# integritychain/fips204

Measured on AMD Instinct MI355X. Metric: ML-DSA-65 verifies/sec per GPU (batched); % HBM roofline, higher is better.
Workload: dtype int32; 1 GPU; ml_dsa_65 batch=65536 whole verify on FIPS 204 wire formats; batch_per_gpu=65536, parallelism=batch-split x1

## Files before the change

### fips204_amd/vfy/vfy.hip

```cpp
#include <hip/hip_runtime.h>
#include <stdint.h>
#include <string.h>

#include <mutex>
#include <string>
#include <vector>

#include "../../include/mldsa_vfy.h"
#include "../layer/layer_dev.h"
#include "../layer/layer_host.h"
#include "../csrc/challenge_dev.h"
#include "../csrc/ntt_wave.h"
#include "../csrc/sampler_dev.h"
#include "../csrc/tables.h"
#include "../csrc/verify_dev.h"
#include "keccak180.h"
#include "vfy_parts.h"

namespace mldsa_vfy {

using mldsa::FWD_TW;
using mldsa::INV_TW;
using mldsa::N;
using mldsa::SHAKE256_RATE;
using mldsa::SWAVES;
using mldsa::Twiddle;
using mldsa::load_le32;
using mldsa::static_for;

#ifndef MLDSA_VFY_EA_WAVES
#define MLDSA_VFY_EA_WAVES 5
#endif
template <int K, int L>
__global__ __launch_bounds__(64 * SWAVES) __attribute__((amdgpu_waves_per_eu(MLDSA_VFY_EA_WAVES, MLDSA_VFY_EA_WAVES))) void k_expand_a(const uint8_t* __restrict__ rho, size_t rho_stride,
                                                                                                    const uint32_t* __restrict__ key_idx,
                                                                                                    int32_t* __restrict__ a_hat, size_t n_ops,
                                                                                                    uint32_t n_keys) {
    const int lane = threadIdx.x & 63;
    const size_t g = (size_t)blockIdx.x * (64 * SWAVES) + threadIdx.x;
    const size_t wave_base = g - lane;
    const size_t n_streams = n_ops * (size_t)(K * L);
    const bool valid = g < n_streams;
    const size_t op = valid ? g / (K * L) : 0;
    const int rs = valid ? (int)(g % (K * L)) : 0;
    const int r = rs / L, sidx = rs % L;
    KeccakState st;
    size_t key = key_idx ? key_idx[op] : op;
    if (n_keys && key >= n_keys) key = 0;
    mldsa::expand_a_seed(st, rho + key * rho_stride, sidx, r);
    rej_ntt_poly_lane_direct180(st, a_hat, wave_base, lane, valid);
}

__global__ __launch_bounds__(256) void k_unpack_a(const uint32_t* __restrict__ packed, int32_t* __restrict__ out, size_t n_polys) {
    const size_t poly = (size_t)blockIdx.x * 4 + (threadIdx.x >> 6);
    if (poly >= n_polys) return;
    const int lane = threadIdx.x & 63;
    const uint32_t* p = packed + poly * mldsa::PACKED_POLY_DWORDS + 3 * lane;
    reinterpret_cast<int4*>(out + poly * N)[lane] = mldsa::unpack24(mldsa::Packed3{p[0], p[1], p[2]});
}

__global__ __launch_bounds__(256) void k_sanitize_keys(const uint32_t* __restrict__ key_idx, uint32_t n_keys, size_t n_ops,
                                                       uint32_t* __restrict__ safe, int32_t* __restrict__ bad) {
    const size_t i = (size_t)blockIdx.x * 256 + threadIdx.x;
    if (i >= n_ops) return;
    const uint32_t k = key_idx[i];
    safe[i] = k < n_keys ? k : 0u;
    bad[i] = k < n_keys ? 0 : 2;
}

constexpr int MU_BLK_STRIDE = 35;
__global__ __launch_bounds__(64) void k_mu(const uint8_t* __restrict__ tr, size_t tr_stride, const uint32_t* __restrict__ key_idx, int mode,
                                           const uint8_t* __restrict__ msgs, const uint64_t* __restrict__ msg_off,
                                           const uint8_t* __restrict__ ctxs, const uint64_t* __restrict__ ctx_off, uint8_t* __restrict__ mu,
                                           size_t mu_stride, int32_t* __restrict__ ctx_bad, const int32_t* __restrict__ key_bad, size_t n_ops,
                                           size_t op0, size_t n_call) {
    __shared__ uint32_t blk[64 * MU_BLK_STRIDE];
    const int lane = threadIdx.x;
    const size_t op = (size_t)blockIdx.x * 64 + lane;
    const bool valid = op < n_ops;
    uint32_t* row = blk + lane * MU_BLK_STRIDE;
    uint8_t* rowb = reinterpret_cast<uint8_t*>(row);

    const uint8_t *trp = nullptr, *mp = nullptr, *cp = nullptr;
    size_t mlen = 0, clen = 0;
    bool live = false;
    if (valid) {
        trp = tr + (key_idx ? key_idx[op] : op) * tr_stride;
        const uint64_t m0 = msg_off[op0 + op], m1 = msg_off[op0 + op + 1];
        bool bad_off = !(msg_off[0] <= m0 && m0 <= m1 && m1 <= msg_off[n_call]);
        mp = msgs + m0;
        mlen = (size_t)(m1 - m0);
        bad_off |= mlen != 0 && msgs == nullptr;
        if (ctx_off) {
            const uint64_t c0 = ctx_off[op0 + op], c1 = ctx_off[op0 + op + 1];
            bad_off |= !(ctx_off[0] <= c0 && c0 <= c1 && c1 <= ctx_off[n_call]);
            cp = ctxs + c0;
            clen = (size_t)(c1 - c0);
            bad_off |= clen != 0 && ctxs == nullptr;
        }
        const int flag = bad_off ? 2 : clen > 255 ? 1 : (key_bad ? key_bad[op] : 0);
        ctx_bad[op] = flag;
        live = !bad_off && clen <= 255;
        if (!live) mlen = clen = 0;
    }
    const size_t pre = (mode == MLDSA_MODE_INTERNAL) ? 0 : 2 + clen;
    const size_t total = live ? 64 + pre + mlen : 0;
    const size_t my_blocks = live ? total / SHAKE256_RATE + 1 : 0;
    size_t max_blocks = my_blocks;
#pragma unroll
    for (int m = 32; m >= 1; m >>= 1) {
        const size_t o = (size_t)__shfl_xor((unsigned long long)max_blocks, m);
        max_blocks = o > max_blocks ? o : max_blocks;
    }
    KeccakState st;
    mldsa::keccak_zero(st);
    for (size_t b = 0; b < max_blocks; b++) {
        if (b < my_blocks) {
            const size_t base = b * SHAKE256_RATE;
            auto byte_at = [&](size_t pos) -> uint8_t {
                if (pos < total) {
                    if (pos < 64) return trp[pos];
                    if (pos < 64 + pre) {
                        const size_t q = pos - 64;
                        return q == 0 ? (uint8_t)(mode == MLDSA_MODE_PREHASH ? 1 : 0) : q == 1 ? (uint8_t)clen : cp[q - 2];
                    }
                    return mp[pos - 64 - pre];
                }
                return pos == total ? (uint8_t)0x1F : (uint8_t)0;
            };
            for (int i = 0; i < SHAKE256_RATE / 4; i++) {
                const size_t pos = base + 4 * (size_t)i;
                uint32_t v;
                if (pos + 4 <= 64) v = load_le32(trp + pos);
                else if (pos >= 64 + pre && pos + 4 <= total) v = load_le32(mp + (pos - 64 - pre));
                else if (pos > total) v = 0;
                else v = (uint32_t)byte_at(pos) | ((uint32_t)byte_at(pos + 1) << 8) | ((uint32_t)byte_at(pos + 2) << 16) | ((uint32_t)byte_at(pos + 3) << 24);
                row[i] = v;
            }
            if (b == my_blocks - 1) rowb[SHAKE256_RATE - 1] |= 0x80;
            static_for<0, 17>([&](auto wc) {
                constexpr int W = decltype(wc)::value;
                st.lo[W] ^= row[2 * W];
                st.hi[W] ^= row[2 * W + 1];
            });
            mldsa::keccak_f1600(st);
        }
    }
    if (valid) {
        uint32_t* out = reinterpret_cast<uint32_t*>(mu + op * mu_stride);
#pragma unroll
        for (int i = 0; i < 8; i++) {
            out[2 * i] = st.lo[i];
            out[2 * i + 1] = st.hi[i];
        }
    }
}

template <int CT>
__global__ __launch_bounds__(64) void k_sample_in_ball(const uint8_t* __restrict__ c_tilde, size_t ct_stride, int tau, uint32_t* __restrict__ c_out,
                                                       size_t n_ops) {
    __shared__ uint32_t c_lds[64 * mldsa::SIB_C_STRIDE];
    __shared__ uint32_t b_lds[64 * mldsa::SIB_BLK_STRIDE];
    const int lane = threadIdx.x;
    const size_t wave_base = (size_t)blockIdx.x * 64;
    const size_t op = wave_base + lane;
    const bool valid = op < n_ops;
    KeccakState st;
    mldsa::keccak_zero(st);
    if (valid) mldsa::absorb_words<CT / 8>(st, c_tilde + op * ct_stride);
    mldsa::shake_pad<SHAKE256_RATE, CT>(st);
    mldsa::sample_in_ball_lane(st, tau, valid, c_lds + lane * mldsa::SIB_C_STRIDE, b_lds + lane * mldsa::SIB_BLK_STRIDE);
    mldsa::wave_lds_sync();
    for (int row = 0; row < 64; row++) {
        if (wave_base + row >= n_ops) break;
        const uint8_t* cb = reinterpret_cast<const uint8_t*>(c_lds + row * mldsa::SIB_C_STRIDE);
        c_out[(wave_base + row) * 64 + lane] =
            (uint32_t)cb[lane] | ((uint32_t)cb[64 + lane] << 8) | ((uint32_t)cb[128 + lane] << 16) | ((uint32_t)cb[192 + lane] << 24);
    }
}

template <int CTRL>
__device__ __forceinline__ int32_t dpp_all(int32_t v) {
    return __builtin_amdgcn_update_dpp(0, v, CTRL, 0xF, 0xF, true);
}

template <int M>
__device__ __forceinline__ void swap_pair(int32_t& x, int32_t& y, int lane) {
    if constexpr (M >= 4) {
        mldsa::swap_pair<M>(x, y, lane);
    } else {
        constexpr int CTRL = M == 2 ? 0x4E : 0xB1;
        const int32_t px = dpp_all<CTRL>(x), py = dpp_all<CTRL>(y);
        const bool up = (lane & M) != 0;
        x = up ? py : x;
        y = up ? y : px;
    }
}
template <int M>
__device__ __forceinline__ void xchg_hi(int32_t r[4], int lane) {
    swap_pair<M>(r[0], r[2], lane);
    swap_pair<M>(r[1], r[3], lane);
}
template <int M>
__device__ __forceinline__ void xchg_lo(int32_t r[4], int lane) {
    swap_pair<M>(r[0], r[1], lane);
    swap_pair<M>(r[2], r[3], lane);
}

template <class TW>
__device__ __forceinline__ void ntt_fwd_wave(int32_t r[4], const TW& tw, int lane) {
    using mldsa::bf_ct;
    bf_ct(r[0], r[2], mldsa::ZF1);
    bf_ct(r[1], r[3], mldsa::ZF1);
    bf_ct(r[0], r[1], mldsa::ZF2);
    bf_ct(r[2], r[3], mldsa::ZF3);
    xchg_hi<32>(r, lane);
    bf_ct(r[0], r[2], tw.get(0));
    bf_ct(r[1], r[3], tw.get(1));
    xchg_lo<16>(r, lane);
    bf_ct(r[0], r[1], tw.get(2));
    bf_ct(r[2], r[3], tw.get(3));
    xchg_hi<8>(r, lane);
    bf_ct(r[0], r[2], tw.get(4));
    bf_ct(r[1], r[3], tw.get(5));
    xchg_lo<4>(r, lane);
    bf_ct(r[0], r[1], tw.get(6));
    bf_ct(r[2], r[3], tw.get(7));
    xchg_hi<2>(r, lane);
    bf_ct(r[0], r[2], tw.get(8));
    bf_ct(r[1], r[3], tw.get(9));
    xchg_lo<1>(r, lane);
    bf_ct(r[0], r[1], tw.get(10));
    bf_ct(r[2], r[3], tw.get(11));
}
template <class TW>
__device__ __forceinline__ void ntt_inv_wave(int32_t r[4], const TW& tw, int lane, int32_t f) {
    using mldsa::bf_gs;
    bf_gs(r[0], r[1], tw.get(0));
    bf_gs(r[2], r[3], tw.get(1));
    bf_gs(r[0], r[2], tw.get(2));
    bf_gs(r[1], r[3], tw.get(3));
    xchg_lo<1>(r, lane);
    bf_gs(r[0], r[1], tw.get(4));
    bf_gs(r[2], r[3], tw.get(5));
    xchg_hi<2>(r, lane);
    bf_gs(r[0], r[2], tw.get(6));
    bf_gs(r[1], r[3], tw.get(7));
    xchg_lo<4>(r, lane);
    bf_gs(r[0], r[1], tw.get(8));
    bf_gs(r[2], r[3], tw.get(9));
    xchg_hi<8>(r, lane);
    bf_gs(r[0], r[2], tw.get(10));
    bf_gs(r[1], r[3], tw.get(11));
    xchg_lo<16>(r, lane);
    bf_gs(r[0], r[1], tw.get(12));
    bf_gs(r[2], r[3], tw.get(13));
    xchg_hi<32>(r, lane);
    const int32_t zf = (int32_t)((((int64_t)mldsa::ZI1 * f) % mldsa::Q) * mldsa::RINV_MOD_Q % mldsa::Q);
#pragma unroll
    for (int k = 0; k < 2; k++) {
        const int32_t a = r[k], b = r[k + 2];
        r[k] = mldsa::caddq(mldsa::mont_mul(a + b, f));
        r[k + 2] = mldsa::caddq(mldsa::mont_mul(a - b, zf));
    }
}

template <bool G2HI>
__device__ __forceinline__ void pack_w1_strided(const uint32_t v[4], uint8_t* dst, int lane) {
    if constexpr (G2HI) {
        uint32_t d[4];
#pragma unroll
        for (int k = 0; k < 4; k++) d[k] = v[k] << (4 * (lane & 7));
#pragma unroll
        for (int k = 0; k < 4; k++) d[k] |= (uint32_t)dpp_all<0xB1>((int32_t)d[k]);
#pragma unroll
        for (int k = 0; k < 4; k++) d[k] |= (uint32_t)dpp_all<0x4E>((int32_t)d[k]);
        const uint32_t d01 = (lane & 1) ? d[1] : d[0], d23 = (lane & 1) ? d[3] : d[2];
        uint32_t mine = (lane & 2) ? d23 : d01;
        mine |= (uint32_t)__builtin_amdgcn_update_dpp(0, (int32_t)mine, 0x104, 0xF, 0xF, true);
        if (!(lane & 4)) mldsa::store_row(reinterpret_cast<uint32_t*>(dst) + 8 * (lane & 3) + (lane >> 3), mine);
    } else {
#pragma unroll
        for (int k = 0; k < 4; k++) {
            const uint32_t n1 = (uint32_t)dpp_all<0xB1>((int32_t)v[k]);
            const uint32_t pair = (lane & 1) ? 0u : (v[k] | (n1 << 6));
            const uint32_t n2 = (uint32_t)dpp_all<0x4E>((int32_t)pair);
            if (!(lane & 3)) {
                const uint32_t q24 = pair | (n2 << 12);
                uint8_t* d = dst + 48 * k + 3 * (lane >> 2);
                d[0] = (uint8_t)q24; d[1] = (uint8_t)(q24 >> 8); d[2] = (uint8_t)(q24 >> 16);
            }
        }
    }
}

constexpr int VW = 4;
template <int K, int L, int GB, bool G2HI, int MINW>
__global__ __launch_bounds__(64 * VW) __attribute__((amdgpu_waves_per_eu(MINW))) void k_verify_main(
    const uint32_t* __restrict__ a_hat, const uint8_t* __restrict__ sigs, size_t sig_len, int ctilde_len, const uint32_t* __restrict__ c,
    const int32_t* __restrict__ t1, const uint32_t* __restrict__ key_idx, size_t key_base, int32_t* __restrict__ hvalid, int omega,
    uint8_t* __restrict__ w1, size_t w1_stride, int32_t* __restrict__ znorm, int32_t zbound, size_t n_ops, const Twiddle* __restrict__ fwd_tab,
    const Twiddle* __restrict__ inv_tab) {
    using mldsa::Packed3;
    constexpr int CB = GB + 1;
    constexpr int BITS = G2HI ? 4 : 6;
    __shared__ int4 zh[VW][L + 1][64];
    __shared__ uint32_t hint_lds[VW][mldsa::HINT_LDS_DWORDS];
    __shared__ Twiddle tw_lds[(FWD_TW + INV_TW) * 64];
    const int lane = threadIdx.x & 63;
    const int wave = __builtin_amdgcn_readfirstlane(threadIdx.x >> 6);
    for (int i = threadIdx.x; i < FWD_TW * 64; i += 64 * VW) tw_lds[i] = fwd_tab[i];
    for (int i = threadIdx.x; i < INV_TW * 64; i += 64 * VW) tw_lds[FWD_TW * 64 + i] = inv_tab[i];
    __syncthreads();
    const mldsa::LdsTw ftw{tw_lds, lane};
    const mldsa::LdsTw itw{tw_lds + FWD_TW * 64, lane};
    const uint32_t wid = blockIdx.x * VW + wave, n_waves = gridDim.x * VW;

    for (size_t op = wid; op < n_ops; op += n_waves) {
        unsigned ul = (unsigned)lane;
        asm volatile("" : "+v"(ul));
        const size_t key = key_idx ? (size_t)__builtin_amdgcn_readfirstlane((int)key_idx[op]) : key_base + op;
        const Packed3* arow = reinterpret_cast<const Packed3*>(a_hat + (op * K * (size_t)L) * mldsa::PACKED_POLY_DWORDS);
        const int4* trow = reinterpret_cast<const int4*>(t1 + (key * K) * (size_t)N);
        Packed3 av[L];
#pragma unroll
        for (int j = 0; j < L; j++) av[j] = mldsa::load_row<mldsa::NT_A_VERIFY>(&arow[(unsigned)(j * 64) + ul]);
        int4 tv = trow[ul];
        const uint8_t* zsrc = sigs + op * sig_len + ctilde_len;
        const mldsa::HintBytes hbytes = mldsa::hint_load(zsrc + L * (32 * CB), omega, K, (int)ul);
        bool zbad = false;
#pragma unroll 1
        for (int j = 0; j <= L; j++) {
            asm volatile("" ::: "memory");
            int32_t r[4];
            if (j < L) {
                const uint8_t* src = zsrc + (size_t)j * (32 * CB);
                int32_t mx = 0;
#pragma unroll
                for (int k = 0; k < 4; k++) {
                    r[k] = mldsa::y_from_raw<CB>(mldsa::y_raw_dword<CB, mldsa::NT_ZC>(src, k, (int)ul), (int)ul);
                    const int32_t a = r[k] < 0 ? -r[k] : r[k];
                    mx = a > mx ? a : mx;
                }
                zbad |= mx >= zbound;
            } else {
                const uint32_t d = mldsa::load_once<mldsa::NT_ZC>(c + op * 64 + ul);
                r[0] = (int8_t)(d & 0xFF); r[1] = (int8_t)((d >> 8) & 0xFF); r[2] = (int8_t)((d >> 16) & 0xFF); r[3] = (int8_t)(d >> 24);
            }
            mldsa_vfy::ntt_fwd_wave(r, ftw, lane);
            if (j == L) {
#pragma unroll
                for (int k = 0; k < 4; k++) r[k] = mldsa::mont_mul(r[k], -1);
            }
            zh[wave][j][lane] = make_int4(r[0], r[1], r[2], r[3]);
        }
        const bool hint_ok = mldsa::hint_unpack_wave<K>(hbytes, omega, hint_lds[wave], (int)ul);
        if (lane == 0) {
            znorm[op] = __ballot(zbad) != 0ull ? 0x7fffffff : 0;
            hvalid[op] = hint_ok ? 1 : 0;
        }
        auto row = [&](int i, const Packed3 (&a_cur)[L], const int4& t_cur, Packed3 (&a_nxt)[L], int4& t_nxt, bool more) {
            const int4 cv = zh[wave][L][lane];
            int64_t acc64[4] = {(int64_t)cv.x * t_cur.x, (int64_t)cv.y * t_cur.y, (int64_t)cv.z * t_cur.z, (int64_t)cv.w * t_cur.w};
#pragma unroll
            for (int j = 0; j < L; j++) {
                const int4 zv = zh[wave][j][lane];
                const int4 a4 = mldsa::unpack24(a_cur[j]);
                acc64[0] += (int64_t)a4.x * zv.x;
                acc64[1] += (int64_t)a4.y * zv.y;
                acc64[2] += (int64_t)a4.z * zv.z;
                acc64[3] += (int64_t)a4.w * zv.w;
            }
            int32_t acc[4];
            if (more) {
#pragma unroll
                for (int j = 0; j < L; j++) a_nxt[j] = mldsa::load_row<mldsa::NT_A_VERIFY>(&arow[(unsigned)(((i + 1) * L + j) * 64) + ul]);
                t_nxt = trow[(unsigned)((i + 1) * 64) + ul];
            }
#pragma unroll
            for (int k = 0; k < 4; k++) acc[k] = mldsa::mont_reduce64(acc64[k]);
            mldsa_vfy::ntt_inv_wave(acc, itw, lane, mldsa::F_MONT2);
            const uint32_t* hrow = hint_lds[wave] + 24 + i * 8 + (ul >> 5);
            uint8_t* dst = w1 + op * w1_stride + (size_t)i * (32 * BITS);
            uint32_t v[4];
#pragma unroll
            for (int k = 0; k < 4; k++) {
                const uint32_t h = (hrow[2 * k] >> (ul & 31)) & 1u;
                v[k] = (uint32_t)mldsa::use_hint<G2HI>((int32_t)h, acc[k]);
            }
            pack_w1_strided<G2HI>(v, dst, lane);
        };
        static_assert(K % 2 == 0, "the row loop runs two rows a trip");
        Packed3 aw[L];
        int4 tw2;
#pragma unroll 1
        for (int i = 0; i < K; i += 2) {
            asm volatile("" ::: "memory");
            row(i, av, tv, aw, tw2, true);
            asm volatile("" ::: "memory");
            row(i + 1, aw, tw2, av, tv, i + 2 < K);
        }
    }
}

constexpr int CWAVES = 4;
constexpr int CBLOCK = 64 * CWAVES;
template <int OUT>
__global__ __launch_bounds__(CBLOCK) void k_ctilde_verdict(const uint8_t* __restrict__ mu_w1, size_t mw, const uint8_t* __restrict__ sigs, size_t sig_len,
                                                           const int32_t* __restrict__ znorm, int32_t zbound, const int32_t* __restrict__ hvalid,
                                                           const int32_t* __restrict__ ctx_bad, uint8_t* __restrict__ ok, size_t n_ops) {
    __shared__ uint32_t tiles[CWAVES * 64 * mldsa::H_STRIDE];
    __shared__ unsigned long long ptr_a[CWAVES * 64];
    const int lane = threadIdx.x & 63, wave = threadIdx.x >> 6;
    uint32_t* tile = tiles + wave * 64 * mldsa::H_STRIDE;
    const size_t base_op = (size_t)blockIdx.x * CBLOCK;
    if (base_op >= n_ops) return;
    const size_t op = base_op + threadIdx.x;
    const bool valid = op < n_ops;
    const size_t opc = valid ? op : base_op;
    ptr_a[wave * 64 + lane] = (unsigned long long)(mu_w1 + opc * mw);
    mldsa::wave_lds_sync_c();
    KeccakState st;
    mldsa::shake256_2_absorb<true>(st, tile, ptr_a + wave * 64, ptr_a + wave * 64, (int)mw, 0, 0, 0, lane);
    if (!valid) return;
    const uint8_t* c0 = sigs + op * sig_len;
    uint32_t diff = 0;
    static_for<0, OUT / 8>([&](auto wc) {
        constexpr int W = decltype(wc)::value;
        diff |= (st.lo[W] ^ load_le32(c0 + 8 * W)) | (st.hi[W] ^ load_le32(c0 + 8 * W + 4));
    });
    ok[op] = (uint8_t)(diff == 0 && znorm[op] < zbound && hvalid[op] && !ctx_bad[op]);
}

}

namespace {

using namespace mldsa_layer;
using namespace mldsa_vfy;

struct DevState {
    int dev = -1;
    int n_cu = 256;
    hipStream_t ea = nullptr, vm = nullptr;
    std::vector<hipEvent_t> ev;
    Twiddle *fwd = nullptr, *inv = nullptr;
    bool prof_on = false;
    std::vector<hipEvent_t> prof_ev;
    std::vector<const char*> prof_name;
    size_t prof_used = 0;
};

std::mutex g_mutex;
std::vector<DevState*> g_states;
size_t g_part_ops = 0;

size_t part_ops() { return g_part_ops ? g_part_ops : (size_t)MLDSA_VFY_PART_OPS; }

int dev_state(const char* fn, int dev, DevState** out) {
    for (DevState* d : g_states)
        if (d->dev == dev) {
            *out = d;
            return MLDSA_OK;
        }
    DevState* d = new DevState;
    d->dev = dev;
    int cu = 0;
    if (hipDeviceGetAttribute(&cu, hipDeviceAttributeMultiprocessorCount, dev) == hipSuccess && cu > 0) d->n_cu = cu;
    const std::vector<mldsa::HostTwiddle> f = mldsa::gen_fwd_lane_twiddles(), i = mldsa::gen_inv_lane_twiddles();
    hipError_t e = hipStreamCreateWithFlags(&d->ea, hipStreamNonBlocking);
    if (e == hipSuccess) e = hipStreamCreateWithFlags(&d->vm, hipStreamNonBlocking);
    if (e == hipSuccess) e = hipMalloc(&d->fwd, f.size() * sizeof(Twiddle));
    if (e == hipSuccess) e = hipMalloc(&d->inv, i.size() * sizeof(Twiddle));
    if (e == hipSuccess) e = hipMemcpy(d->fwd, f.data(), f.size() * sizeof(Twiddle), hipMemcpyHostToDevice);
    if (e == hipSuccess) e = hipMemcpy(d->inv, i.data(), i.size() * sizeof(Twiddle), hipMemcpyHostToDevice);
    if (e != hipSuccess || f.size() != (size_t)FWD_TW * 64 || i.size() != (size_t)INV_TW * 64) {
        if (d->ea) (void)hipStreamDestroy(d->ea);
        if (d->vm) (void)hipStreamDestroy(d->vm);
        if (d->fwd) (void)hipFree(d->fwd);
        if (d->inv) (void)hipFree(d->inv);
        delete d;
        (void)hipGetLastError();
        return e != hipSuccess ? hip_failed(fn, "creating the library's streams and tables", e)
                               : fail(MLDSA_ERR_DEVICE, std::string(fn) + ": the core's twiddle tables have another shape");
    }
    g_states.push_back(d);
    *out = d;
    return MLDSA_OK;
}

struct Events {
    DevState* d;
    size_t used = 0;
    hipError_t err = hipSuccess;
    explicit Events(DevState* d_) : d(d_) {}
    hipEvent_t next() {
        if (used == d->ev.size()) {
            hipEvent_t e = nullptr;
            const hipError_t rc = hipEventCreateWithFlags(&e, hipEventDisableTiming);
            if (rc != hipSuccess) {
                err = rc;
                return nullptr;
            }
            d->ev.push_back(e);
        }
        return d->ev[used++];
    }
};

constexpr size_t PROF_MAX_PAIRS = 4096;
struct ProfScope {
    DevState* d;
    hipStream_t s;
    long idx = -1;
    ProfScope(DevState* d_, hipStream_t s_, const char* name) : d(d_), s(s_) {
        if (!d->prof_on || d->prof_used >= PROF_MAX_PAIRS) return;
        if (d->prof_used * 2 + 2 > d->prof_ev.size()) {
            hipEvent_t a = nullptr, b = nullptr;
            if (hipEventCreate(&a) != hipSuccess) return;
            if (hipEventCreate(&b) != hipSuccess) {
                (void)hipEventDestroy(a);
                return;
            }
            d->prof_ev.push_back(a);
            d->prof_ev.push_back(b);
            d->prof_name.push_back(name);
        } else {
            d->prof_name[d->prof_used] = name;
        }
        idx = (long)d->prof_used++;
        (void)hipEventRecord(d->prof_ev[2 * idx], s);
    }
    ~ProfScope() {
        if (idx >= 0) (void)hipEventRecord(d->prof_ev[2 * idx + 1], s);
    }
};

#define VFY_HIP(call, what)                                     \
    do {                                                        \
        const hipError_t e_ = (call);                           \
        if (e_ != hipSuccess) return hip_failed(fn, what, e_);  \
    } while (0)

#define VFY_BY_SET(set, M)              \
    do {                                \
        if ((set) == MLDSA_44) M(4, 4, 17, false, 32, 5); \
        else if ((set) == MLDSA_65) M(6, 5, 19, true, 48, 4); \
        else M(8, 7, 19, true, 64, 4);  \
    } while (0)

unsigned stream_blocks(size_t n_streams) { return (unsigned)((n_streams + 64 * SWAVES - 1) / (64 * SWAVES)); }

void launch_expand_a(int set, const uint8_t* rho, const uint32_t* key_idx, int32_t* a_hat, size_t n, uint32_t n_keys, hipStream_t s) {
    mldsa_params p;
    (void)mldsa_get_params(set, &p);
    const dim3 grid(stream_blocks(n * (size_t)(p.k * p.l))), block(64 * SWAVES);
#define VFY_EA(KK, LL, GB, G2, CT, MW) hipLaunchKernelGGL((k_expand_a<KK, LL>), grid, block, 0, s, rho, (size_t)32, key_idx, a_hat, n, n_keys)
    VFY_BY_SET(set, VFY_EA);
#undef VFY_EA
}

struct Call {
    int set, mode;
    mldsa_params p;
    const uint8_t *rho, *tr;
    const int32_t* t1;
    size_t n_keys;
    const uint32_t* key_idx;
    const uint8_t* msgs;
    const uint64_t* msg_off;
    const uint8_t* ctxs;
    const uint64_t* ctx_off;
    const uint8_t* sigs;
    uint8_t* ok;
    size_t n_ops;
};

int enqueue(const char* fn, DevState* d, const Call& c, uint8_t* scratch, hipStream_t s) {
    const mldsa_params& p = c.p;
    const PartPlan plan(c.n_ops, part_ops());
    const Carve cv = carve(p.k, p.l, (size_t)p.w1_len, plan);
    const size_t mw = 64 + (size_t)p.w1_len;
    uint32_t* c8 = reinterpret_cast<uint32_t*>(scratch + cv.c);
    int32_t* znorm = reinterpret_cast<int32_t*>(scratch + cv.znorm);
    int32_t* hvalid = reinterpret_cast<int32_t*>(scratch + cv.hvalid);
    int32_t* ctx_bad = reinterpret_cast<int32_t*>(scratch + cv.ctx_bad);
    int32_t* key_bad = reinterpret_cast<int32_t*>(scratch + cv.key_bad);
    uint32_t* kidx = reinterpret_cast<uint32_t*>(scratch + cv.kidx);
    uint8_t* mu_w1 = scratch + cv.mu_w1;
    const size_t sig_len = (size_t)p.sig_len;

    const OrderPlan order = order_plan(plan.n_parts());
    const hipStream_t lanes[N_LANES] = {s, d->ea, d->vm};
    Events evs(d);
    std::vector<hipEvent_t> ev(order.n_events);
    for (hipEvent_t& e : ev) e = evs.next();
    if (evs.err != hipSuccess) return hip_failed(fn, "creating an event", evs.err);

    for (const Step& st : order.steps) {
        const hipStream_t q = lanes[st.lane];
        if (st.act == ACT_RECORD) {
            VFY_HIP(hipEventRecord(ev[st.n], q), (std::string("recording ") + st.what).c_str());
            continue;
        }
        if (st.act == ACT_WAIT) {
            VFY_HIP(hipStreamWaitEvent(q, ev[st.n], 0), (std::string("waiting for ") + st.what).c_str());
            continue;
        }
        const Part part = plan.at(st.n);
        const size_t o = part.first, n = part.count;
        const size_t key_base = c.key_idx ? 0 : o;
        int32_t* a_hat = reinterpret_cast<int32_t*>(scratch + cv.ring[part.half]);
        const uint8_t* sg = c.sigs + o * sig_len;
        const uint32_t* kp = c.key_idx ? kidx + o : nullptr;
        const int32_t* kb = c.key_idx ? key_bad + o : nullptr;
        switch (st.stage) {
        case STAGE_EXPAND_A: {
            ProfScope ps(d, q, "expand_a");
            launch_expand_a(c.set, c.rho + key_base * 32, c.key_idx ? c.key_idx + o : nullptr, a_hat, n, c.key_idx ? (uint32_t)c.n_keys : 0u, q);
            break;
        }
        case STAGE_FRONT: {
            if (c.key_idx)
                hipLaunchKernelGGL(k_sanitize_keys, dim3((unsigned)((n + 255) / 256)), dim3(256), 0, q, c.key_idx + o, (uint32_t)c.n_keys, n, kidx + o, key_bad + o);
            {
                ProfScope ps(d, q, "mu");
                hipLaunchKernelGGL(k_mu, dim3((unsigned)((n + 63) / 64)), dim3(64), 0, q, c.tr + key_base * 64, (size_t)64, kp, c.mode, c.msgs, c.msg_off, c.ctxs,
                                   c.ctx_off, mu_w1 + o * mw, mw, ctx_bad + o, kb, n, o, c.n_ops);
            }
            {
                ProfScope ps(d, q, "sample_in_ball");
                const dim3 grid((unsigned)((n + 63) / 64)), block(64);
#define VFY_SIB(KK, LL, GB, G2, CT, MW) hipLaunchKernelGGL((k_sample_in_ball<CT>), grid, block, 0, q, sg, sig_len, p.tau, c8 + o * 64, n)
                VFY_BY_SET(c.set, VFY_SIB);
#undef VFY_SIB
            }
            break;
        }
        case STAGE_VERIFY_MAIN: {
            ProfScope ps(d, q, "verify_main");
            const size_t need = (n + VW - 1) / VW, cap = (size_t)d->n_cu * 16;
            const dim3 grid((unsigned)(need < cap ? need : cap)), block(64 * VW);
#define VFY_VM(KK, LL, GB, G2, CT, MW)                                                                                                         \
    hipLaunchKernelGGL((k_verify_main<KK, LL, GB, G2, MW>), grid, block, 0, q, reinterpret_cast<const uint32_t*>(a_hat), sg, sig_len,          \
                       p.ctilde_len, c8 + o * 64, c.t1, kp, key_base, hvalid + o, p.omega, mu_w1 + o * mw + 64, mw, znorm + o, p.gamma1 - p.beta, n, \
                       d->fwd, d->inv)
            VFY_BY_SET(c.set, VFY_VM);
#undef VFY_VM
            break;
        }
        default: {
            ProfScope ps(d, q, "ctilde_hash");
            const dim3 grid((unsigned)((n + CBLOCK - 1) / CBLOCK)), block(CBLOCK);
#define VFY_CT(KK, LL, GB, G2, CT, MW)                                                                                                    \
    hipLaunchKernelGGL((k_ctilde_verdict<CT>), grid, block, 0, q, mu_w1 + o * mw, mw, sg, sig_len, znorm + o, p.gamma1 - p.beta, hvalid + o, \
                       ctx_bad + o, c.ok + o, n)
            VFY_BY_SET(c.set, VFY_CT);
#undef VFY_CT
            break;
        }
        }
        LAYER_LAUNCHED(st.what);
    }
    return MLDSA_OK;
}

void drain(DevState* d) {
    (void)hipStreamSynchronize(d->ea);
    (void)hipStreamSynchronize(d->vm);
    (void)hipGetLastError();
}

size_t scratch_bytes_of(int set, size_t n_ops) {
    mldsa_params p;
    if (mldsa_get_params(set, &p) != MLDSA_OK || n_ops > MLDSA_VFY_MAX_OPS) return 0;
    return carve(p.k, p.l, (size_t)p.w1_len, PartPlan(n_ops, part_ops())).bytes;
}

}

extern "C" {

int mldsa_vfy_abi_version(void) { return MLDSA_VFY_ABI_VERSION; }

const char* mldsa_vfy_last_error(void) { return g_err.c_str(); }

size_t mldsa_vfy_scratch_bytes(int set, size_t n_ops) {
    std::lock_guard<std::mutex> lk(g_mutex);
    return scratch_bytes_of(set, n_ops);
}

size_t mldsa_vfy_set_part_ops(size_t part) {
    std::lock_guard<std::mutex> lk(g_mutex);
    const size_t before = part_ops();
    g_part_ops = part;
    return before;
}

int mldsa_vfy_verify(mldsa_ctx* ctx, int set, int mode, const uint8_t* rho, const uint8_t* tr, const int32_t* t1_d2_hat_mont, size_t n_keys,
                     const uint32_t* key_idx, const uint8_t* msgs, const uint64_t* msg_off, const uint8_t* ctxs, const uint64_t* ctx_off,
                     const uint8_t* sigs, uint8_t* ok, size_t n_ops, void* scratch, size_t scratch_bytes, void* stream) {
    const char* fn = "mldsa_vfy_verify";
    Call c;
    const int rc = check_common(fn, ctx, set, n_ops, MLDSA_VFY_MAX_OPS, "MLDSA_VFY_MAX_OPS ops", &c.p);
    if (rc != MLDSA_OK) return rc;
    if (mode != MLDSA_MODE_PURE && mode != MLDSA_MODE_INTERNAL && mode != MLDSA_MODE_PREHASH)
        return fail(MLDSA_ERR_PARAM, std::string(fn) + ": bad mode");
    if (n_ops == 0) return MLDSA_OK;
    if (!rho || !tr || !t1_d2_hat_mont || !msg_off || !sigs || !ok) return fail(MLDSA_ERR_PARAM, std::string(fn) + ": NULL pointer");
    if (key_idx ? n_keys == 0 : n_keys < n_ops) return fail(MLDSA_ERR_PARAM, std::string(fn) + ": n_keys does not cover the batch");
    if (n_keys > 0xFFFFFFFFu) n_keys = 0xFFFFFFFFu;
    if (!aligned(t1_d2_hat_mont, 16)) return fail(MLDSA_ERR_PARAM, std::string(fn) + ": t1_d2_hat_mont must be 16-byte aligned");
    if (!scratch || !aligned(scratch, 256)) return fail(MLDSA_ERR_PARAM, std::string(fn) + ": scratch is NULL or not 256-byte aligned");
    LAYER_ON_DEVICE(ctx);
    std::lock_guard<std::mutex> lk(g_mutex);
    if (scratch_bytes < scratch_bytes_of(set, n_ops))
        return fail(MLDSA_ERR_NOMEM, std::string(fn) + ": scratch is below mldsa_vfy_scratch_bytes(set, n_ops)");
    DevState* d = nullptr;
    const int src = dev_state(fn, dev_, &d);
    if (src != MLDSA_OK) return src;
    c.set = set; c.mode = mode; c.rho = rho; c.tr = tr; c.t1 = t1_d2_hat_mont; c.n_keys = n_keys; c.key_idx = key_idx; c.msgs = msgs;
    c.msg_off = msg_off; c.ctxs = ctxs; c.ctx_off = ctx_off; c.sigs = sigs; c.ok = ok; c.n_ops = n_ops;
    const int erc = enqueue(fn, d, c, static_cast<uint8_t*>(scratch), (hipStream_t)stream);
    if (erc != MLDSA_OK) drain(d);
    return erc;
}

int mldsa_vfy_expand_a(mldsa_ctx* ctx, int set, const uint8_t* rho, int32_t* a_hat, size_t n_ops, void* stream) {
    const char* fn = "mldsa_vfy_expand_a";
    mldsa_params p;
    const int rc = check_common(fn, ctx, set, n_ops, MLDSA_VFY_MAX_OPS, "MLDSA_VFY_MAX_OPS ops", &p);
    if (rc != MLDSA_OK) return rc;
    if (n_ops == 0) return MLDSA_OK;
    if (!rho || !a_hat) return fail(MLDSA_ERR_PARAM, std::string(fn) + ": NULL pointer");
    if (!aligned(a_hat, 16)) return fail(MLDSA_ERR_PARAM, std::string(fn) + ": a_hat must be 16-byte aligned");
    LAYER_ON_DEVICE(ctx);
    hipStream_t s = (hipStream_t)stream;
    const size_t n_polys = n_ops * (size_t)(p.k * p.l);
    void* packed = nullptr;
    VFY_HIP(hipMalloc(&packed, n_polys * PACKED_POLY_BYTES), "allocating the packed rows");
    launch_expand_a(set, rho, nullptr, static_cast<int32_t*>(packed), n_ops, 0u, s);
    hipLaunchKernelGGL(k_unpack_a, dim3((unsigned)((n_polys + 3) / 4)), dim3(256), 0, s, static_cast<const uint32_t*>(packed), a_hat, n_polys);
    hipError_t e = hipGetLastError();
    const hipError_t se = hipStreamSynchronize(s);
    if (e == hipSuccess) e = se;
    (void)hipFree(packed);
    return e == hipSuccess ? MLDSA_OK : hip_failed(fn, "ExpandA and unpack", e);
}

int mldsa_vfy_profile_enable(mldsa_ctx* ctx, int on) {
    const char* fn = "mldsa_vfy_profile_enable";
    if (!ctx) return fail(MLDSA_ERR_PARAM, std::string(fn) + ": NULL context");
    LAYER_ON_DEVICE(ctx);
    std::lock_guard<std::mutex> lk(g_mutex);
    DevState* d = nullptr;
    const int rc = dev_state(fn, dev_, &d);
    if (rc != MLDSA_OK) return rc;
    d->prof_on = on != 0;
    if (!d->prof_on) d->prof_used = 0;
    return MLDSA_OK;
}

int mldsa_vfy_profile_report(mldsa_ctx* ctx, char* buf, size_t buf_len) {
    const char* fn = "mldsa_vfy_profile_report";
    if (!ctx) return fail(MLDSA_ERR_PARAM, std::string(fn) + ": NULL context");
    if (!buf || buf_len <= 2) return fail(MLDSA_ERR_PARAM, std::string(fn) + ": bad argument");
    LAYER_ON_DEVICE(ctx);
    std::lock_guard<std::mutex> lk(g_mutex);
    DevState* d = nullptr;
    const int rc = dev_state(fn, dev_, &d);
    if (rc != MLDSA_OK) return rc;
    VFY_HIP(hipDeviceSynchronize(), "waiting for the device");
    struct Acc { const char* name; double ms; size_t calls; };
    std::vector<Acc> acc;
    for (size_t i = 0; i < d->prof_used; i++) {
        float ms = 0.f;
        if (hipEventElapsedTime(&ms, d->prof_ev[2 * i], d->prof_ev[2 * i + 1]) != hipSuccess) {
            (void)hipGetLastError();
            continue;
        }
        bool found = false;
        for (auto& a : acc)
            if (strcmp(a.name, d->prof_name[i]) == 0) {
                a.ms += ms;
                a.calls++;
                found = true;
                break;
            }
        if (!found) acc.push_back({d->prof_name[i], ms, 1});
    }
    std::string out = "{";
    for (size_t i = 0; i < acc.size(); i++)
        out += std::string(i ? ", " : "") + "\"" + acc[i].name + "\": {\"ms\": " + std::to_string(acc[i].ms) + ", \"calls\": " + std::to_string(acc[i].calls) + "}";
    out += "}";
    if (out.size() + 1 > buf_len) return fail(MLDSA_ERR_PARAM, std::string(fn) + ": buffer too small");
    memcpy(buf, out.c_str(), out.size() + 1);
    d->prof_used = 0;
    return MLDSA_OK;
}

}
```

### fips204_amd/vfy/vfy_parts.h

```cpp
#pragma once
#include <stddef.h>
#include <stdint.h>

#include <vector>

namespace mldsa_vfy {

constexpr size_t PACKED_POLY_BYTES = 768;
constexpr size_t CARVE_ALIGN = 256;

struct Part {
    size_t first = 0, count = 0;
    int half = 0;
};

struct PartPlan {
    size_t n_ops, part;
    PartPlan(size_t n_ops_, size_t part_) : n_ops(n_ops_), part(part_ ? part_ : 1) {}
    size_t n_parts() const { return n_ops / part + (n_ops % part ? 1 : 0); }
    size_t halves() const { return n_parts() > 1 ? 2 : n_parts(); }
    size_t half_ops() const { return n_ops < part ? n_ops : part; }
    Part at(size_t i) const {
        Part p;
        p.first = i * part;
        p.count = n_ops - p.first < part ? n_ops - p.first : part;
        p.half = (int)(i & 1);
        return p;
    }
};

struct Carve {
    size_t ring[2];
    size_t ring_bytes;
    size_t c;
    size_t znorm, hvalid, ctx_bad, key_bad, kidx;
    size_t mu_w1;
    size_t bytes;
};

inline size_t carve_up(size_t x) { return (x + CARVE_ALIGN - 1) / CARVE_ALIGN * CARVE_ALIGN; }

inline Carve carve(int k, int l, size_t w1_len, const PartPlan& plan) {
    Carve c;
    size_t at = 0;
    auto take = [&at](size_t bytes) {
        const size_t here = at;
        at += carve_up(bytes);
        return here;
    };
    c.ring_bytes = plan.half_ops() * (size_t)(k * l) * PACKED_POLY_BYTES;
    c.ring[0] = take(c.ring_bytes);
    c.ring[1] = plan.halves() > 1 ? take(c.ring_bytes) : c.ring[0];
    c.c = take(plan.n_ops * 256);
    c.znorm = take(plan.n_ops * 4);
    c.hvalid = take(plan.n_ops * 4);
    c.ctx_bad = take(plan.n_ops * 4);
    c.key_bad = take(plan.n_ops * 4);
    c.kidx = take(plan.n_ops * 4);
    c.mu_w1 = take(plan.n_ops * (64 + w1_len));
    c.bytes = at + CARVE_ALIGN;
    return c;
}

enum Lane { LANE_CALLER = 0, LANE_EA = 1, LANE_VM = 2, N_LANES = 3 };
enum Action { ACT_RECORD, ACT_WAIT, ACT_LAUNCH };
enum Stage { STAGE_EXPAND_A = 0, STAGE_FRONT = 1, STAGE_VERIFY_MAIN = 2, STAGE_CTILDE = 3, N_STAGES = 4 };

struct Step {
    Lane lane;
    Action act;
    Stage stage;
    size_t n;
    const char* what;
};

struct OrderPlan {
    std::vector<Step> steps;
    size_t n_events = 0;
};

struct StageLanes {
    Lane expand_a, arith, front;
};
inline StageLanes lanes_of_call(size_t n_parts) {
    return n_parts == 1 ? StageLanes{LANE_CALLER, LANE_CALLER, LANE_VM} : StageLanes{LANE_EA, LANE_VM, LANE_CALLER};
}

inline OrderPlan order_plan(size_t n_parts, const StageLanes& on) {
    OrderPlan o;
    if (n_parts == 0) return o;
    const size_t none = (size_t)-1;
    auto put = [&o](Lane lane, Action act, Stage stage, size_t n, const char* what) { o.steps.push_back(Step{lane, act, stage, n, what}); };
    const size_t fork = o.n_events++;
    bool forked[N_LANES] = {true, false, false};
    auto reach = [&](Lane lane, Stage stage) {
        if (!forked[lane]) put(lane, ACT_WAIT, stage, fork, "the fork");
        forked[lane] = true;
    };
    auto record = [&](Lane from, Lane to, Stage stage, const char* what) {
        if (from == to) return none;
        put(from, ACT_RECORD, stage, o.n_events, what);
        return o.n_events++;
    };
    auto wait = [&](Lane to, size_t event, Stage stage, const char* what) {
        if (event == none) return;
        put(to, ACT_WAIT, stage, event, what);
        forked[to] = true;
    };
    put(LANE_CALLER, ACT_RECORD, STAGE_EXPAND_A, fork, "the fork");
    std::vector<size_t> used(n_parts, none);
    for (size_t p = 0; p < n_parts; p++) {
        if (p >= 2) wait(on.expand_a, used[p - 2], STAGE_EXPAND_A, "the ring half");
        reach(on.expand_a, STAGE_EXPAND_A);
        put(on.expand_a, ACT_LAUNCH, STAGE_EXPAND_A, p, "k_expand_a launch");
        const size_t ready = record(on.expand_a, on.arith, STAGE_EXPAND_A, "ExpandA's end");
        reach(on.front, STAGE_FRONT);
        put(on.front, ACT_LAUNCH, STAGE_FRONT, p, "front launch");
        const size_t front = record(on.front, on.arith, STAGE_FRONT, "the front's end");
        wait(on.arith, ready, STAGE_EXPAND_A, "ExpandA");
        wait(on.arith, front, STAGE_FRONT, "the front");
        reach(on.arith, STAGE_VERIFY_MAIN);
        put(on.arith, ACT_LAUNCH, STAGE_VERIFY_MAIN, p, "k_verify_main launch");
        if (p + 2 < n_parts) used[p] = record(on.arith, on.expand_a, STAGE_VERIFY_MAIN, "the end of the ring half's use");
        put(on.arith, ACT_LAUNCH, STAGE_CTILDE, p, "k_ctilde_verdict launch");
    }
    wait(LANE_CALLER, record(on.arith, LANE_CALLER, STAGE_CTILDE, "the join"), STAGE_CTILDE, "the join");
    return o;
}

inline OrderPlan order_plan(size_t n_parts) { return order_plan(n_parts, lanes_of_call(n_parts)); }

}
```

Baseline: 40.40 million verifies/s.

## Use branch-free UseHint, immediate-offset A/t1 addressing, and peel challenge NTT

Replaces the library UseHint with branch-free versions that divide by multiply-shift and handle wraparound arithmetically for both gamma2 variants. Addresses A-hat and t1 rows through a base pointer centred mid-row so the per-polynomial offsets can fit in load instruction immediate offsets, cutting address arithmetic. Peels the challenge-polynomial NTT out of the z loop to remove per-iteration branches, and pins the prefetched A registers with an asm barrier to shape scheduling. The custom UseHint constants must be exact over the full input range.

Result: no change. 40.69 million verifies/s, median of 6 (+0.7%).

```diff
diff --git a/fips204_amd/vfy/vfy.hip b/fips204_amd/vfy/vfy.hip
--- a/fips204_amd/vfy/vfy.hip
+++ b/fips204_amd/vfy/vfy.hip
@@ -266,6 +266,12 @@
 }
 
 template <bool G2HI>
+__device__ __forceinline__ uint32_t use_hint(uint32_t h, int32_t r) {
+    if constexpr (G2HI) return (uint32_t)use_hint_32((int32_t)h, r);
+    else return (uint32_t)use_hint_88((int32_t)h, r);
+}
+
+template <bool G2HI>
 __device__ __forceinline__ void pack_w1_strided(const uint32_t v[4], uint8_t* dst, int lane) {
     if constexpr (G2HI) {
         uint32_t d[4];
@@ -295,6 +301,7 @@
 }
 
 constexpr int VW = 4;
+typedef uint32_t u32x3 __attribute__((ext_vector_type(3)));
 template <int K, int L, int GB, bool G2HI, int MINW>
 __global__ __launch_bounds__(64 * VW) __attribute__((amdgpu_waves_per_eu(MINW))) void k_verify_main(
     const uint32_t* __restrict__ a_hat, const uint8_t* __restrict__ sigs, size_t sig_len, int ctilde_len, const uint32_t* __restrict__ c,
@@ -320,39 +327,45 @@
         unsigned ul = (unsigned)lane;
         asm volatile("" : "+v"(ul));
         const size_t key = key_idx ? (size_t)__builtin_amdgcn_readfirstlane((int)key_idx[op]) : key_base + op;
-        const Packed3* arow = reinterpret_cast<const Packed3*>(a_hat + (op * K * (size_t)L) * mldsa::PACKED_POLY_DWORDS);
-        const int4* trow = reinterpret_cast<const int4*>(t1 + (key * K) * (size_t)N);
+        constexpr int ROW_BYTES = 4 * mldsa::PACKED_POLY_DWORDS;
+        constexpr int AMID = (L / 2) * ROW_BYTES;
+        static_assert(AMID < 4096 && (L - 1) * ROW_BYTES - AMID < 4096, "the polynomials of a row within the immediate offset");
+        const char* abase = reinterpret_cast<const char*>(a_hat + (op * K * (size_t)L) * mldsa::PACKED_POLY_DWORDS) + AMID;
+        const char* tbase = reinterpret_cast<const char*>(t1 + (key * K) * (size_t)N);
+        auto a_at = [&](int i, int j) {
+            return reinterpret_cast<const Packed3*>(abase + (size_t)i * (L * ROW_BYTES) + (size_t)(12u * ul) + (j * ROW_BYTES - AMID));
+        };
+        auto t_at = [&](int i) { return *reinterpret_cast<const int4*>(tbase + (size_t)i * (4 * N) + (size_t)(16u * ul)); };
         Packed3 av[L];
 #pragma unroll
-        for (int j = 0; j < L; j++) av[j] = mldsa::load_row<mldsa::NT_A_VERIFY>(&arow[(unsigned)(j * 64) + ul]);
-        int4 tv = trow[ul];
+        for (int j = 0; j < L; j++) av[j] = mldsa::load_row<mldsa::NT_A_VERIFY>(a_at(0, j));
+        int4 tv = t_at(0);
         const uint8_t* zsrc = sigs + op * sig_len + ctilde_len;
         const mldsa::HintBytes hbytes = mldsa::hint_load(zsrc + L * (32 * CB), omega, K, (int)ul);
         bool zbad = false;
 #pragma unroll 1
-        for (int j = 0; j <= L; j++) {
+        for (int j = 0; j < L; j++) {
             asm volatile("" ::: "memory");
-            int32_t r[4];
-            if (j < L) {
-                const uint8_t* src = zsrc + (size_t)j * (32 * CB);
-                int32_t mx = 0;
-#pragma unroll
-                for (int k = 0; k < 4; k++) {
-                    r[k] = mldsa::y_from_raw<CB>(mldsa::y_raw_dword<CB, mldsa::NT_ZC>(src, k, (int)ul), (int)ul);
-                    const int32_t a = r[k] < 0 ? -r[k] : r[k];
-                    mx = a > mx ? a : mx;
-                }
-                zbad |= mx >= zbound;
-            } else {
-                const uint32_t d = mldsa::load_once<mldsa::NT_ZC>(c + op * 64 + ul);
-                r[0] = (int8_t)(d & 0xFF); r[1] = (int8_t)((d >> 8) & 0xFF); r[2] = (int8_t)((d >> 16) & 0xFF); r[3] = (int8_t)(d >> 24);
-            }
+            const uint8_t* src = zsrc + (size_t)j * (32 * CB);
+            int32_t r[4], mx = 0;
+#pragma unroll
+            for (int k = 0; k < 4; k++) {
+                r[k] = mldsa::y_from_raw<CB>(mldsa::y_raw_dword<CB, mldsa::NT_ZC>(src, k, (int)ul), (int)ul);
+                const int32_t a = r[k] < 0 ? -r[k] : r[k];
+                mx = a > mx ? a : mx;
+            }
+            zbad |= mx >= zbound;
             mldsa_vfy::ntt_fwd_wave(r, ftw, lane);
-            if (j == L) {
-#pragma unroll
-                for (int k = 0; k < 4; k++) r[k] = mldsa::mont_mul(r[k], -1);
-            }
             zh[wave][j][lane] = make_int4(r[0], r[1], r[2], r[3]);
+        }
+        {
+            asm volatile("" ::: "memory");
+            const uint32_t d = mldsa::load_once<mldsa::NT_ZC>(c + op * 64 + ul);
+            int32_t r[4] = {(int8_t)(d & 0xFF), (int8_t)((d >> 8) & 0xFF), (int8_t)((d >> 16) & 0xFF), (int8_t)(d >> 24)};
+            mldsa_vfy::ntt_fwd_wave(r, ftw, lane);
+#pragma unroll
+            for (int k = 0; k < 4; k++) r[k] = mldsa::mont_mul(r[k], -1);
+            zh[wave][L][lane] = make_int4(r[0], r[1], r[2], r[3]);
         }
         const bool hint_ok = mldsa::hint_unpack_wave<K>(hbytes, omega, hint_lds[wave], (int)ul);
         if (lane == 0) {
@@ -374,8 +387,8 @@
             int32_t acc[4];
             if (more) {
 #pragma unroll
-                for (int j = 0; j < L; j++) a_nxt[j] = mldsa::load_row<mldsa::NT_A_VERIFY>(&arow[(unsigned)(((i + 1) * L + j) * 64) + ul]);
-                t_nxt = trow[(unsigned)((i + 1) * 64) + ul];
+                for (int j = 0; j < L; j++) a_nxt[j] = mldsa::load_row<mldsa::NT_A_VERIFY>(a_at(i + 1, j));
+                t_nxt = t_at(i + 1);
             }
 #pragma unroll
             for (int k = 0; k < 4; k++) acc[k] = mldsa::mont_reduce64(acc64[k]);
@@ -386,7 +399,7 @@
 #pragma unroll
             for (int k = 0; k < 4; k++) {
                 const uint32_t h = (hrow[2 * k] >> (ul & 31)) & 1u;
-                v[k] = (uint32_t)mldsa::use_hint<G2HI>((int32_t)h, acc[k]);
+                v[k] = mldsa_vfy::use_hint<G2HI>(h, acc[k]);
             }
             pack_w1_strided<G2HI>(v, dst, lane);
         };
@@ -396,6 +409,12 @@
 #pragma unroll 1
         for (int i = 0; i < K; i += 2) {
             asm volatile("" ::: "memory");
+#pragma unroll
+            for (int j = 0; j < L; j++) {
+                u32x3 t = {av[j].a, av[j].b, av[j].c};
+                asm volatile("" : "+v"(t));
+                av[j] = Packed3{t.x, t.y, t.z};
+            }
             row(i, av, tv, aw, tw2, true);
             asm volatile("" ::: "memory");
             row(i + 1, aw, tw2, av, tv, i + 2 < K);
diff --git a/fips204_amd/vfy/vfy_parts.h b/fips204_amd/vfy/vfy_parts.h
--- a/fips204_amd/vfy/vfy_parts.h
+++ b/fips204_amd/vfy/vfy_parts.h
@@ -60,6 +60,25 @@
     c.mu_w1 = take(plan.n_ops * (64 + w1_len));
     c.bytes = at + CARVE_ALIGN;
     return c;
+}
+
+constexpr int32_t USE_HINT_Q = 8380417;
+
+constexpr int32_t use_hint_32(int32_t h, int32_t r) {
+    constexpr int32_t G2 = (USE_HINT_Q - 1) / 32;
+    const uint32_t n = (uint32_t)r + (G2 - 1);
+    const int32_t r1 = (int32_t)(((uint64_t)n * 2149582851u) >> 50);
+    const int32_t m = ((int32_t)n - r1 * (2 * G2) - G2) >> 31;
+    return (r1 + ((h ^ m) - m)) & 15;
+}
+
+constexpr int32_t use_hint_88(int32_t h, int32_t r) {
+    constexpr int32_t G2 = (USE_HINT_Q - 1) / 88;
+    const uint32_t n = (uint32_t)r + (G2 - 1);
+    const int32_t r1 = (int32_t)(((uint64_t)n * 2955676419u) >> 49);
+    const int32_t m = ((int32_t)n - r1 * (2 * G2) - G2) >> 31;
+    const int32_t u = r1 + 44 + ((h ^ m) - m);
+    return u - 44 * ((u * 745) >> 15);
 }
 
 enum Lane { LANE_CALLER = 0, LANE_EA = 1, LANE_VM = 2, N_LANES = 3 };
```
